# AlexIoannides/bodywork-mlops-demo

Hardware: NVIDIA H100
Metric: train rows/sec (N x 128 least-squares fit) (higher is better)
Workload: dtype bf16x2 (hi+lo) MMA operands, f32 accumulate, f64 fold+solve

## Files before the change

bodywork-mlops-demo_b200/csrc/b2_internal.cuh:

```cuda
#pragma once
#include <cuda.h>
#include <cuda_bf16.h>
#include <cuda_runtime.h>
#include <stdint.h>
#include <stdio.h>
#include <string.h>

#include <type_traits>

#include "../../include/b2gram.h"

namespace b2 {

constexpr int kMaxD = B2_MAX_D;
constexpr int kMaxS = kMaxD + 2;
constexpr int kKernelEventPairs = 64;
constexpr int kMaxRanks = 8;
constexpr size_t kXchgSlotDoubles = (size_t)kMaxS * kMaxS;
constexpr size_t kXchgDataDoubles = 2 * kMaxRanks * kXchgSlotDoubles;
constexpr size_t kXchgBytes = kXchgDataDoubles * sizeof(double) + 256;

constexpr int kTcRows = 64;
constexpr int kTcM = 128;
constexpr int kTcEMax = 16;
// ... 108 lines not shown
constexpr int kLcYbar = kLcC + kMaxD * kMaxClasses;
constexpr int kLcSum = kLcYbar + kMaxClasses;
constexpr int kLcPart = 2 * kMaxAlphas;
constexpr int kLcDoubles = kLcSum + kLcPart;

constexpr int kMnHead = 32;
constexpr int kMnClasses = 0;
constexpr int kMnCoef = kMaxClasses;
constexpr int kMnStep = kMnCoef + kMaxClasses * (kMaxD + 1);
constexpr int kMnOpDoubles = kMnStep + kMaxClasses * (kMaxD + 1);

constexpr int kDaHead = 8;
constexpr int kDaPart = kDaHead + kMaxD * kMaxD;
constexpr int kDaClasses = 0;
constexpr int kDaWeights = kMaxClasses;
constexpr int kDaMeans = 2 * kMaxClasses;
constexpr int kDaSums = kDaMeans + kMaxClasses * kMaxD;
constexpr int kDaDoubles = kDaSums + kDaPart;

constexpr int kQdClasses = 0;
constexpr int kQdMeans = kMaxClasses;
constexpr int kQdConst = kQdMeans + kMaxClasses * kMaxD;
constexpr int kQdW = kQdConst + kMaxClasses;
constexpr int kQdSums = kQdW + kMaxClasses * kMaxD * kMaxD;
constexpr int kQdCounts = kQdSums + kMaxClasses * kMaxD * kMaxD;
constexpr int kQdDoubles = kQdCounts + kMaxClasses + 8;
constexpr int64_t kQdSpan = 1 << 24;
constexpr int kQdChunk = 8192;
constexpr int kQdMaxChunks = (int)(kQdSpan / kQdChunk);
constexpr size_t kQdScratchBytes = sizeof(int) * (size_t)kQdSpan;
constexpr int kQdItemsPerSm = 2;
constexpr int kQdHdCorrect = 0;
constexpr int kQdHdNItems = 4;
constexpr int kQdHdCounts = 5;
constexpr int kQdHdStart = 8;
constexpr int kQdHdFirstItem = kQdHdStart + kMaxClasses + 1;
constexpr int kQdHdCnt = 80;
constexpr int kQdHdItems = kQdHdCnt + kQdMaxChunks * (kMaxClasses + 3);
static_assert(kQdHdFirstItem + kMaxClasses + 1 <= kQdHdCnt, "qda header");
int qda_max_items(const b2_ctx* ctx);

constexpr int kMaxFolds = 254;
int launch_fold_ranges(b2_ctx* ctx, const uint8_t* fold_of_row, int64_t n, int n_folds, unsigned long long* range);
int launch_fold_sum(b2_ctx* ctx, const double* folds, int n_folds, int d, double* S);

inline int narrow_dp(int d) { return d <= 1 ? 1 : d <= 2 ? 2 : d <= 4 ? 4 : d <= 8 ? 8 : 16; }

void set_error(const char* fmt, ...);

#define B2_CUDA(call)                                                                      \
  do {                                                                                     \
    cudaError_t e_ = (call);                                                               \
    if (e_ != cudaSuccess) {                                                               \
      b2::set_error("%s failed: %s (%s:%d)", #call, cudaGetErrorString(e_), __FILE__, __LINE__); \
      return B2_E_CUDA;                                                                    \
    }                                                                                      \
  } while (0)

}

struct b2_ctx {
  int device = 0;
  int sm_count = 0;
  size_t hbm_bytes = 0;
  char name[128] = {0};
  cudaStream_t stream = nullptr;
  cudaStream_t copy_stream = nullptr;
  cudaEvent_t ev_t0 = nullptr, ev_t1 = nullptr;
  cudaEvent_t ev_k[b2::kKernelEventPairs][2];
  int k_pairs = 0;
  int64_t launches = 0;

  int kernel_mode = B2_KERNEL_AUTO;
  int drain_rows = 8192;
  int precision = B2_PRECISION_SPLIT;

  int d = 0;
  double* S = nullptr;

  double* tc_part = nullptr;
  double* tc_red = nullptr;
  float* shift = nullptr;
  bool solve_attr_set = false;
  double* solve_host = nullptr;
  struct TmCache {
    const void* X = nullptr; const float* y = nullptr; const uint8_t* mask = nullptr;
    int64_t n = 0, ldx = 0; int d = 0, x_dtype = -1;
    int y_map_2d = 0, m_map_2d = 0;
    alignas(64) unsigned char tmX[128], tmY[128], tmM[128];
  } tm_cache;
  double* simt_part = nullptr;
  int simt_ctas = 0;
  double* score_part = nullptr;
  int score_ctas = 0;
  double* coef_dev = nullptr;
  double* grad_part = nullptr;
  double* refine = nullptr;
  double* loo = nullptr;
  double* loo_part = nullptr;
  double* enet = nullptr;
  size_t enet_doubles = 0;
  double* folds = nullptr;
  size_t folds_doubles = 0;
  int n_folds = 0;
  int folds_d = 0;
  unsigned long long* fold_range = nullptr;
  double* glm = nullptr;
  double* glm_part = nullptr;
  double* cls = nullptr;
  double* loo_cls = nullptr;
  double* mn_op = nullptr;
  double* mn_sum = nullptr;
  size_t mn_sum_doubles = 0;
  double* mn_part = nullptr;
  size_t mn_part_doubles = 0;
  double* disc = nullptr;
  double* disc_part = nullptr;
  double* qda = nullptr;
  int* qda_hd = nullptr;
  void* qda_scratch = nullptr;
  double* qda_part = nullptr;
  double* coef_host = nullptr;
  cudaEvent_t ev_coef[2] = {nullptr, nullptr};
  int coef_slot = 0;
  long long* synth_count = nullptr;
  double* solve_out = nullptr;
  void* stage_x[2] = {nullptr, nullptr};
  float* stage_y[2] = {nullptr, nullptr};
  uint8_t* stage_m[2] = {nullptr, nullptr};
  size_t stage_bytes_x = 0;
  int64_t stage_rows = 0;
  cudaEvent_t ev_copied[2] = {nullptr, nullptr};
  cudaEvent_t ev_consumed[2] = {nullptr, nullptr};
  bool ev_consumed_valid[2] = {false, false};
  char* row_out[2] = {nullptr, nullptr};
  size_t row_out_bytes = 0;
  void* bounce[2] = {nullptr, nullptr};
  cudaEvent_t ev_bounce[2] = {nullptr, nullptr};
  bool s_zero_pending = false;
  void* comm = nullptr;
  int n_ranks = 1, rank = 0;
  double* xchg = nullptr;
  double* xchg_peer[8] = {nullptr};
  bool p2p_ready = false;
  bool p2p_local = false;
  unsigned int xchg_epoch = 0;
  unsigned long long xchg_timeout_ns = 10000000000ull;
  bool xchg_pending = false;
  unsigned int* xchg_status_host = nullptr;
  unsigned int* tc_sync = nullptr;
  int fused_fits = 0;
  int sm_limit = 0;
  bool sm_limit_auto = false;
};

namespace b2 {

inline double* score_totals(const b2_ctx* ctx) { return ctx->score_part + (size_t)ctx->score_ctas * kNStats; }

template <typename... P, typename... A>
int launch_smem(void (*kernel)(P...), int grid, int threads, uint32_t smem, cudaStream_t stream, A... args) {
  B2_CUDA(cudaFuncSetAttribute(kernel, cudaFuncAttributeMaxDynamicSharedMemorySize, smem));
  kernel<<<grid, threads, smem, stream>>>(args...);
  B2_CUDA(cudaGetLastError());
  return B2_OK;
}
// ... 123 lines not shown
```

bodywork-mlops-demo_b200/csrc/gram_tc.cu:

```cuda
#include <cuda_bf16.h>
#include <stdlib.h>

#include "b2_internal.cuh"
#include "b2_ptx.cuh"
#include "b2_shift.cuh"
#include "b2_xchg.cuh"

namespace b2 {
namespace {

constexpr int kConsumerWGs = 2;
constexpr int kXformWarps = 8;
constexpr int kThreads = 128 * (kConsumerWGs + 2);
constexpr int kFirstXformWarp = 4 * kConsumerWGs;
constexpr int kTmaWarp = kFirstXformWarp;
constexpr int kEWarp = kFirstXformWarp + 1;
static_assert(kFirstXformWarp + kXformWarps == kThreads / 32, "warp roles");
constexpr int kProducers = kXformWarps;
constexpr int kConsumerWarps = 4 * kConsumerWGs;
constexpr int kKGroups = kTcRows / 8;
constexpr uint32_t kRawStageBytes = kTcRows * kMaxD * 4;
constexpr uint32_t kOpSBO = 128;
constexpr uint32_t kOpLBO = (16 + 2 + 16) * kOpSBO;
constexpr uint32_t kOpEOff = 16 * kOpSBO;
// ... 265 lines not shown
  auto P = [&](int acc, int i, int j) { return __ldcg(red + tc_part_index(acc, i, j, ew)); };
  auto s1 = [&](int i) {
    double t = 0.0;
    for (int blk = 0; blk < pack; ++blk) {
      const int r = blk * d + i, e = kTcM + 3 * blk;
      t += d2 ? P(0, r, e) + P(1, r, e) : P(0, r, e);
    }
    return t;
  };
  auto sxy = [&](int i) {
    double t = 0.0;
    for (int blk = 0; blk < pack; ++blk) {
      const int r = blk * d + i, e = kTcM + 3 * blk;
      t += d2 ? P(0, r, e + 1) + P(0, r, e + 2) + P(1, r, e + 1) + P(1, r, e + 2) : P(0, r, e + 1) + P(0, r, e + 2);
    }
    return t;
  };
  auto G = [&](int i, int j) {
    double g = 0.0;
    for (int blk = 0; blk < pack; ++blk) {
      const int ia = blk * d + i, ib = blk * d + j;
      const double g1 = P(0, min(ia, ib), max(ia, ib));
      g += d2 ? g1 + P(1, ia, ib) + P(1, ib, ia) : g1;
    }
    return g;
  };
  return unshift_entry(a, b, d, c, G, s1, sxy, __ldcg(red + kTcAccElems + 2), __ldcg(red + kTcAccElems + 0),
                       __ldcg(red + kTcAccElems + 1));
}

template <typename T, int DFIX, bool SPLIT, bool RAWB = false, int EW = 8>
__global__ void __launch_bounds__(kThreads, 1)
gram_tc_kernel(const __grid_constant__ CUtensorMap tmX, const __grid_constant__ CUtensorMap tmY,
               const __grid_constant__ CUtensorMap tmM, int y_map_2d, int has_mask, int keep,
               int64_t n_rows, int d_arg, int pack, int d_orig, const float* __restrict__ shift,
               int chunk_tiles, double* __restrict__ part, uint32_t wait_ns, uint32_t dbg_arg) {
#ifdef B2_DEV_KNOBS
  const uint32_t dbg = dbg_arg;
#else
  constexpr uint32_t dbg = 0u;
  (void)dbg_arg;
#endif
  using G = TcGeo<RAWB>;
  constexpr int kRawStages = G::kRawStages, kOpStages = G::kOpStages;
  constexpr uint32_t kOffRaw = G::kOffRaw, kOffOp = G::kOffOp, kOffY = G::kOffY, kOffMask = G::kOffMask;
  const int d = DFIX ? DFIX : d_arg;
  extern __shared__ uint8_t smem_raw[];
  const uint32_t sbase = (smem_u32(smem_raw) + 1023u) & ~1023u;
  uint8_t* smem = smem_raw + (sbase - smem_u32(smem_raw));
  const int warp = threadIdx.x >> 5;
  const int lane = threadIdx.x & 31;

  const uint32_t bar_raw_full = sbase + G::kOffBar;
  const uint32_t bar_raw_empty = bar_raw_full + 8 * kRawStages;
  const uint32_t bar_op_full = bar_raw_empty + 8 * kRawStages;
  const uint32_t bar_op_empty = bar_op_full + 8 * kOpStages;
  float* shift_s = reinterpret_cast<float*>(smem + G::kOffShift);

  const int64_t total_tiles = (n_rows + kTcRows - 1) / kTcRows;
  const int64_t tile_begin = (int64_t)blockIdx.x * total_tiles / gridDim.x;
  const int64_t tile_end = (int64_t)(blockIdx.x + 1) * total_tiles / gridDim.x;
  const int my_tiles = (int)(tile_end - tile_begin);

  if (threadIdx.x == 0) {
    for (int s = 0; s < kRawStages; ++s) {
      mbar_init(bar_raw_full + 8 * s, 1);
      mbar_init(bar_raw_empty + 8 * s, kProducers + (RAWB ? kConsumerWarps : 0));
    }
    for (int s = 0; s < kOpStages; ++s) {
      mbar_init(bar_op_full + 8 * s, kProducers);
      mbar_init(bar_op_empty + 8 * s, kConsumerWarps);
    }
    asm volatile("fence.mbarrier_init.release.cluster;" ::: "memory");
  }
  if (warp == kTmaWarp && lane == 0) {
    tma_prefetch_desc(&tmX);
    tma_prefetch_desc(&tmY);
    if (has_mask) tma_prefetch_desc(&tmM);
  }
  for (uint32_t o = threadIdx.x * 16; o < kOpStages * kOpStageBytes; o += kThreads * 16)
    *reinterpret_cast<uint4*>(smem + kOffOp + o) = make_uint4(0, 0, 0, 0);
  for (int j = threadIdx.x; j <= kMaxD; j += kThreads)
    shift_s[j] = j == kMaxD ? shift[kMaxD] : (j < pack * d_orig ? shift[j % d_orig] : 0.f);
  fence_proxy_async_smem();
  __syncthreads();

  if (warp < kConsumerWarps) {
    asm volatile("setmaxnreg.inc.sync.aligned.u32 %0;" ::"n"(G::kConsumerRegs));
    auto consume = [&](auto wg_c) {
      constexpr int WG = decltype(wg_c)::value;
      constexpr int kF1 = kTcM - 64 * WG;
      constexpr int kF2 = RAWB ? kF1 : kTcM;
      constexpr int kC1 = 64 * WG;
      constexpr int kR1 = (kF1 + EW) / 2, kR2 = (kF2 + EW) / 2;
      float acc1[kR1], acc2[kR2];
      using H = TcSums<DFIX, SPLIT, RAWB, EW, WG>;
      double* my_part = part + (size_t)blockIdx.x * kTcAccElems;
      double sums[H::kRegs > 0 ? H::kRegs : 1];
      const bool on_chip_off = (dbg & 256u) != 0u;
      auto slab_addr = [&](int s, int ln) {
        return sbase + G::kOffSlab + (uint32_t)(((4 * H::kSlabBase + (warp & 3) * H::kSlab + s) * 32 + ln) * 8);
      };
      auto store = [&](auto n_regs, int dst_acc, int col0, bool add, auto val) {
        const int ln = (int)lane_id(), row0 = 64 * WG + 16 * (warp & 3) + (ln >> 2);
#pragma unroll
        for (int r = 0; r < decltype(n_regs)::value; ++r) {
          const int col = col0 + 8 * (r >> 2) + 2 * (ln & 3) + (r & 1), h = (r >> 1) & 1, i = row0 + 8 * h;
          const bool lower = dst_acc == 0 && col < kTcM && i > col;
          const double v = val(r, col, h);
          const bool on_chip = dst_acc == 0 && r >= H::kFirstSlab;
          if (on_chip && r >= H::kFirstReg) {
            double& s = sums[r - H::kFirstReg];
            s = add ? __dadd_rn(s, v) : v;
          } else if (on_chip) {
            const uint32_t a = slab_addr(r - H::kFirstSlab, ln);
            st_shared_f64_if(a, add ? __dadd_rn(ld_shared_f64(a), v) : v, !on_chip_off);
          }
          put_f64(my_part + tc_part_index(dst_acc, i, col, EW), v, add, !lower && (!on_chip || on_chip_off));
        }
      };
      auto flush = [&]() {
        const int ln = (int)lane_id(), row0 = 64 * WG + 16 * (warp & 3) + (ln >> 2);
#pragma unroll
        for (int r = H::kFirstSlab; r < H::kR1; ++r) {
          const int col = kC1 + 8 * (r >> 2) + 2 * (ln & 3) + (r & 1), i = row0 + 8 * ((r >> 1) & 1);
          const double s = r >= H::kFirstReg ? sums[r - H::kFirstReg] : ld_shared_f64(slab_addr(r - H::kFirstSlab, ln));
          put_f64(my_part + tc_part_index(0, i, col, EW), s, false, !(col < kTcM && i > col) && !on_chip_off);
        }
      };
      auto drain = [&](const auto& acc, int dst_acc, int col0, bool add) {
        constexpr int kR = sizeof(acc) / sizeof(float);
        if constexpr (RAWB) {
          constexpr int kF = 2 * kR - EW;
          const double s1[2] = {(double)__shfl_sync(0xffffffffu, acc[kF / 2], lane & ~3),
                                (double)__shfl_sync(0xffffffffu, acc[kF / 2 + 2], lane & ~3)};
          store(std::integral_constant<int, kR>{}, dst_acc, col0, add, [&](int r, int col, int h) {
            return col < kTcM ? (double)acc[r] - (double)shift_s[col] * s1[h] : (double)acc[r];
          });
        } else {
          store(std::integral_constant<int, kR>{}, dst_acc, col0, add, [&](int r, int, int) { return (double)acc[r]; });
        }
      };
      auto release = [&](int tile) {
        mbar_arrive(bar_op_empty + 8 * (tile % kOpStages));
        if constexpr (RAWB) mbar_arrive(bar_raw_empty + 8 * (tile % kRawStages));
      };
      constexpr uint32_t a_off = (uint32_t)WG * 8 * kOpSBO;
      int os = 0, held = -1, in_chunk = 0;
      uint32_t oph = 0;
      bool first_chunk = true;
      for (int it = 0; it < my_tiles; ++it) {
        mbar_wait(bar_op_full + 8 * os, oph, wait_ns);
        const uint32_t op_addr = sbase + kOffOp + os * kOpStageBytes;
        wgmma_fence();
#pragma unroll
        for (int k2 = 0; k2 < kTcRows / 16; ++k2) {
          const uint32_t k_addr = op_addr + k2 * 2 * kOpLBO;
          const uint64_t hi_desc = make_smem_desc(k_addr + a_off), lo_desc = make_smem_desc(k_addr + kOpLoOff + a_off);
          const uint32_t sc1 = (in_chunk > 0 || k2 > 0) ? 1u : 0u, sc2 = (it > 0 || k2 > 0) ? 1u : 0u;
          if constexpr (RAWB) {
            const uint64_t x_desc = make_raw_desc(sbase + kOffRaw + (uint32_t)(it % kRawStages) * kRawStageBytes +
                                                  (uint32_t)WG * kRawBoxBytes + k2 * 16 * 128);
            const uint64_t e_desc = make_smem_desc(k_addr + kOpEOff);
            if (!(dbg & 2u)) {
              wgmma<kF1, 1>(acc1, hi_desc, x_desc, sc1);
              wgmma<EW, 0>(acc1 + kF1 / 2, hi_desc, e_desc, sc1);
            }
            if (SPLIT && !(dbg & 3u)) {
              wgmma<kF2, 1>(acc2, lo_desc, x_desc, sc2);
              wgmma<EW, 0>(acc2 + kF2 / 2, lo_desc, e_desc, sc2);
            }
          } else {
            if (!(dbg & 2u)) wgmma<kF1 + EW, 0>(acc1, hi_desc, make_smem_desc(k_addr + a_off), sc1);
            if (SPLIT && !(dbg & 3u)) wgmma<kF2 + EW, 0>(acc2, lo_desc, make_smem_desc(k_addr), sc2);
          }
        }
        wgmma_commit();
        const bool last = (in_chunk == chunk_tiles - 1) || (it == my_tiles - 1);
        if (last) {
          wgmma_wait<0>();
          fence_regs(acc1);
          if constexpr (SPLIT) fence_regs(acc2);
        } else {
          wgmma_wait<1>();
        }
        if (lane == 0) {
          if (held >= 0) release(held);
          if (last) release(it);
        }
        held = last ? -1 : it;
        if (last) {
          drain(acc1, 0, kC1, !first_chunk);
          first_chunk = false;
          in_chunk = 0;
        } else {
          ++in_chunk;
        }
        if (++os == kOpStages) { os = 0; oph ^= 1; }
      }
      wgmma_wait<0>();
      if constexpr (SPLIT) {
        fence_regs(acc2);
        drain(acc2, RAWB ? 0 : 1, RAWB ? kC1 : 0, RAWB);
      }
      flush();
    };
    if (__shfl_sync(0xffffffffu, warp, 0) >= 4) consume(std::integral_constant<int, 1>{});
    else consume(std::integral_constant<int, 0>{});
  } else {
    asm volatile("setmaxnreg.dec.sync.aligned.u32 %0;" ::"n"(G::kProducerRegs));
    const uint32_t tx = (uint32_t)(kTcRows * d * sizeof(T)) + kTcRows * pack * 4 + (has_mask ? kTcRows * pack : 0);
    auto issue = [&](int j) {
      const int s = j % kRawStages;
      mbar_wait(bar_raw_empty + 8 * s, ((uint32_t)(j / kRawStages) & 1u) ^ 1u, wait_ns);
      const uint32_t full = bar_raw_full + 8 * s;
      mbar_expect_tx(full, tx);
      const int64_t row0 = (tile_begin + j) * kTcRows;
      tma_load_2d(sbase + kOffRaw + s * kRawStageBytes, &tmX, 0, (int)row0, full);
      if constexpr (RAWB) tma_load_2d(sbase + kOffRaw + s * kRawStageBytes + kRawBoxBytes, &tmX, 64, (int)row0, full);
      const int sub0 = (int)row0 * pack;
      if (y_map_2d) tma_load_2d(sbase + kOffY + s * kYStageBytes, &tmY, 0, sub0 >> 2, full);
      else tma_load_1d(sbase + kOffY + s * kYStageBytes, &tmY, sub0, full);
      if (has_mask == 2) tma_load_2d(sbase + kOffMask + s * kMStageBytes, &tmM, 0, sub0 >> 4, full);
      else if (has_mask) tma_load_1d(sbase + kOffMask + s * kMStageBytes, &tmM, sub0, full);
    };
    const bool issuer = warp == kTmaWarp && lane == 0;
    if (issuer)
      for (int j = 0; j < G::kAhead && j < my_tiles; ++j) issue(j);

    const int t = warp - kFirstXformWarp;
    const int nb = (d + 63) >> 6;
    const int i = 64 * (t % nb) + 2 * lane;
    const uint32_t swp = ((uint32_t)lane >> 2) & 1u;
    const uint32_t st_off = (uint32_t)((i >> 3) * kOpSBO + (i & 7) * 16);
    auto esum = [&]() { return sbase + G::kOffESum + 8 * lane_id(); };
    if (warp == kEWarp) { st_shared_f64(esum(), 0.0); st_shared_f64(esum() + 256, 0.0); st_shared_f64(esum() + 512, 0.0); }
    int rs = 0, os = 0;
    uint32_t rph = 0, oph = 0;
    for (int it = 0; it < my_tiles; ++it) {
      if (issuer && it + G::kAhead < my_tiles) issue(it + G::kAhead);
      __syncwarp();
      mbar_wait(bar_raw_full + 8 * rs, rph, wait_ns);
      mbar_wait(bar_op_empty + 8 * os, oph ^ 1, wait_ns);
      const int64_t row0 = (tile_begin + it) * kTcRows;
      const int64_t left = n_rows - row0;
      const int rows_valid = left < kTcRows ? (int)left : kTcRows;
      const bool full_tile = (!has_mask) && (rows_valid == kTcRows);
      const uint32_t raw_addr = sbase + kOffRaw + rs * kRawStageBytes;
      const uint32_t m_addr = sbase + kOffMask + rs * kMStageBytes;
      const uint32_t op_addr = sbase + kOffOp + os * kOpStageBytes;
      if (warp == kEWarp && !(dbg & 192u)) {
        const uint32_t y_addr = sbase + kOffY + rs * kYStageBytes;
        const uint32_t e_addr = op_addr + kOpEOff;
        const float c_y = shift_s[kMaxD];
        float a = 0.f, b = 0.f, c = 0.f;
        for (int half = 0; half < kTcRows / 32; ++half) {
          const int rr = lane + 32 * half;
          const uint32_t dst = e_addr + (rr >> 3) * kOpLBO + (rr & 7) * 2;
          for (int bl = 0; bl < pack; ++bl) {
            const int sub = rr * pack + bl;
            bool use = rr < rows_valid;
            if (use && has_mask) use = (ld_shared_u8(m_addr + sub) == (uint32_t)keep);
            const float yv = use ? ld_shared_f32(y_addr + sub * 4) - c_y : 0.f;
            uint32_t yh, yl;
            split2(yv, 0.f, yh, yl);
            st_shared_u16(dst + (3 * bl) * 16, use ? 0x3F80u : 0u);
            st_shared_u16(dst + (3 * bl + 1) * 16, yh);
            st_shared_u16(dst + (3 * bl + 2) * 16, yl);
            if (RAWB && has_mask && !use) {
              const uint32_t row = raw_addr + (uint32_t)rr * 128;
              const uint32_t z[4] = {0u, 0u, 0u, 0u};
#pragma unroll
              for (int q = 0; q < 8; ++q) { st_shared_v4(row + 16 * q, z); st_shared_v4(row + kRawBoxBytes + 16 * q, z); }
            }
            a += yv;
            b = fmaf(yv, yv, b);
            c += use ? 1.f : 0.f;
          }
        }
        const uint32_t es = esum();
        st_shared_f64(es, ld_shared_f64(es) + (double)a);
        st_shared_f64(es + 256, ld_shared_f64(es + 256) + (double)b);
        st_shared_f64(es + 512, ld_shared_f64(es + 512) + (double)c);
      }
      if (i < d && !(dbg & 128u)) {
        float c_i[2];
        ld_vals_vec<float, 2>(sbase + G::kOffShift + 4 * (uint32_t)i, c_i);
        for (int g = t / nb; g < kKGroups; g += kXformWarps / nb) {
          const int r0 = g * 8;
          float v0[8], v1[8];
          const uint32_t src = raw_addr + (uint32_t)r0 * ((uint32_t)d * sizeof(T)) + (uint32_t)i * sizeof(T);
// ... 213 lines not shown
    if (pack > kMaxPack) pack = kMaxPack;
    if (n_in < (int64_t)2 * kTcRows * pack) pack = 1;
  }
  const int group = pack == 1 ? 1 : (pack == 3 ? 48 : (pack == 5 ? 80 : 16));
  if (pack_out != nullptr) *pack_out = pack;
  return n_in - n_in % group;
}

int launch_gram_tc(b2_ctx* ctx, const void* X, int x_dtype, const float* y, int64_t n_in, int d_in, int64_t ldx_in,
                   const uint8_t* mask, int keep, bool assign, unsigned int scatter_epoch) {
  PFN_encodeTiled encode = get_encode();
  if (encode == nullptr) {
    set_error("cuTensorMapEncodeTiled is not available from the driver");
    return B2_E_CUDA;
  }
  const int es = x_dtype == B2_F32 ? 4 : 2;
  int pack = 1;
  const int64_t n_main = gram_tc_main_rows(n_in, d_in, ldx_in, &pack);
  const int64_t n = n_main / pack;
  const int d = pack > 1 ? 128 : d_in;
  const int d_tensor = d_in * pack;
  const int64_t ldx = ldx_in * pack;
  const int64_t n_y = n_main;
  const bool rawb = x_dtype == B2_BF16 && d_in == 128 && pack == 1;
  CUtensorMap tmX, tmY, tmM;
  b2_ctx::TmCache& tc = ctx->tm_cache;
  const bool cached = tc.X == X && tc.y == y && tc.mask == mask && tc.n == n_in && tc.ldx == ldx_in && tc.d == d_in &&
                      tc.x_dtype == x_dtype;
  if (cached) {
    memcpy(&tmX, tc.tmX, sizeof(tmX)); memcpy(&tmY, tc.tmY, sizeof(tmY)); memcpy(&tmM, tc.tmM, sizeof(tmM));
  } else {
    int y_map_2d = 0, m_map_2d = 0;
    if (int r = encode_maps(encode, X, x_dtype, es, y, n, d_tensor, d, ldx, n_y, pack, mask, rawb, &tmX, &tmY, &tmM, &y_map_2d,
                            &m_map_2d))
      return r;
    tc.X = X; tc.y = y; tc.mask = mask; tc.n = n_in; tc.ldx = ldx_in; tc.d = d_in; tc.x_dtype = x_dtype;
    tc.y_map_2d = y_map_2d; tc.m_map_2d = m_map_2d;
    memcpy(tc.tmX, &tmX, sizeof(tmX)); memcpy(tc.tmY, &tmY, sizeof(tmY)); memcpy(tc.tmM, &tmM, sizeof(tmM));
  }

  const int64_t total_tiles = (n + kTcRows - 1) / kTcRows;
  const int sms = (ctx->sm_limit > 0 && ctx->sm_limit < ctx->sm_count) ? ctx->sm_limit : ctx->sm_count;
  const int grid = (int)(total_tiles < sms ? total_tiles : sms);
  int chunk_tiles = ctx->drain_rows / kTcRows / (rawb ? 4 : 1);
  if (chunk_tiles < 1) chunk_tiles = 1;

#ifdef B2_DEV_KNOBS
  static const uint32_t wait_ns = []() {
    const char* e = getenv("B2_WAIT_HINT_NS");
    return e ? (uint32_t)atoi(e) : 20000u;
  }();
#else
  constexpr uint32_t wait_ns = 20000u;
#endif
#ifdef B2_DEV_KNOBS
  static const uint32_t dbg = []() {
    const char* e = getenv("B2_TC_DEBUG");
    return e ? (uint32_t)atoi(e) : 0u;
  }();
#else
  constexpr uint32_t dbg = 0u;
#endif
  const bool split = ctx->precision == B2_PRECISION_SPLIT;
  const int ew = tc_e_width(pack);
  const bool d2 = split && !rawb;
  decltype(&gram_tc_kernel<float, 0, false>) kernel = nullptr;
  uint32_t smem = TcGeo<false>::kSmemBytes;
  with_rows(x_dtype, X, [&](auto* Xr) {
    using T = row_t<decltype(Xr)>;
    return with_int<0, 1>(split, [&](auto SP) {
      constexpr bool kSplit = decltype(SP)::value;
      if (d != 128) kernel = gram_tc_kernel<T, 0, kSplit>;
      else if (ew == 16) kernel = gram_tc_kernel<T, 128, kSplit, false, 16>;
      else kernel = gram_tc_kernel<T, 128, kSplit>;
      if constexpr (std::is_same_v<T, __nv_bfloat16>) {
        if (rawb) {
          kernel = gram_tc_kernel<T, 128, kSplit, true>;
          smem = TcGeo<true>::kSmemBytes;
        }
      }
      return B2_OK;
    });
  });
  B2_CUDA(cudaFuncSetAttribute(kernel, cudaFuncAttributeMaxDynamicSharedMemorySize, smem));
  const int pair = ctx->k_pairs % kKernelEventPairs;
  B2_CUDA(cudaEventRecord(ctx->ev_k[pair][0], ctx->stream));
  kernel<<<grid, kThreads, smem, ctx->stream>>>(tmX, tmY, tmM, tc.y_map_2d, mask != nullptr ? 1 + tc.m_map_2d : 0, keep,
                                                n, d, pack, d_in, ctx->shift, chunk_tiles, ctx->tc_part, wait_ns, dbg);
  B2_CUDA(cudaGetLastError());
  B2_CUDA(cudaEventRecord(ctx->ev_k[pair][1], ctx->stream));
  ctx->k_pairs += 1;

  TcFinal fin;
  memset(&fin, 0, sizeof(fin));
  fin.assign = assign ? 1 : 0;
  fin.n_ranks = 1;
  if (scatter_epoch != 0) {
    fin.n_ranks = ctx->n_ranks; fin.rank = ctx->rank; fin.epoch = scatter_epoch;
    for (int r = 0; r < kMaxRanks; ++r) fin.peers.p[r] = ctx->xchg_peer[r];
  }
  {
    cudaLaunchConfig_t cfg;
    memset(&cfg, 0, sizeof(cfg));
    cfg.gridDim = dim3(kFinalizeCtas < sms ? kFinalizeCtas : sms);
    cfg.blockDim = dim3(kFinalizeThreads); cfg.dynamicSmemBytes = 0; cfg.stream = ctx->stream;
    cudaLaunchAttribute attr[1];
    attr[0].id = cudaLaunchAttributeCooperative;
    attr[0].val.cooperative = 1;
    cfg.attrs = attr; cfg.numAttrs = 1;
    const double* part_arg = ctx->tc_part;
    const float* shift_arg = ctx->shift;
    B2_CUDA(cudaLaunchKernelEx(&cfg, tc_finalize_kernel, part_arg, grid, ctx->tc_red, shift_arg, d_in, pack, ew,
                               d2 ? 1 : 0, ctx->S, ctx->tc_sync, fin));
  }
  ctx->launches += 2;
  return B2_OK;
}

}
```

bodywork-mlops-demo_b200/csrc/solve.cu:

```cuda
#include "b2_internal.cuh"
#include "b2_xchg.cuh"

namespace b2 {
namespace {

constexpr int kOutIntercept = kMaxD;
constexpr int kOutInfo = kMaxD + 1;
constexpr int kOutRank = kMaxD + 2;
constexpr int kOutSingular = kMaxD + 3;
constexpr int kOutRows = kOutSingular + kMaxD;

struct LdcgStat {
  const double* S;
  __device__ __forceinline__ double operator()(int i) const { return __ldcg(S + i); }
};

template <class Stat>
__device__ void build_normal_equations_of(const Stat& S, int d, double alpha, int fit_intercept,
                                       double* A, double* r, double* mean, double* ybar_out) {
  const int dp = d + 2, pitch = d + 1;
  const double n = S(d * dp + d);
  const double inv_n = n > 0.0 ? 1.0 / n : 0.0;
  double sxy = 0.0;
  if ((int)threadIdx.x < d) {
    const double sx = S(threadIdx.x * dp + d);
    sxy = S(threadIdx.x * dp + d + 1);
    mean[threadIdx.x] = fit_intercept ? sx * inv_n : 0.0;
  }
  const double ybar = fit_intercept ? S(d * dp + d + 1) * inv_n : 0.0;
  __syncthreads();
  if ((int)threadIdx.x < d) r[threadIdx.x] = sxy - n * mean[threadIdx.x] * ybar;
  const int lane = threadIdx.x & 31, warp = threadIdx.x >> 5, nwarps = blockDim.x >> 5;
  for (int i0 = warp; i0 < d; i0 += 2 * nwarps) {
    const int i1 = i0 + nwarps;
    double v[8];
#pragma unroll
    for (int u = 0; u < 4; ++u) {
      const int j = lane + 32 * u;
      v[u] = j < d ? S(i0 * dp + j) : 0.0;
      v[4 + u] = (j < d && i1 < d) ? S(i1 * dp + j) : 0.0;
    }
    const double m0 = mean[i0], m1 = i1 < d ? mean[i1] : 0.0;
#pragma unroll
    for (int u = 0; u < 4; ++u) {
      const int j = lane + 32 * u;
      if (j < d) {
        const double mj = mean[j];
        A[i0 * pitch + j] = v[u] - n * m0 * mj + (i0 == j ? alpha : 0.0);
        if (i1 < d) A[i1 * pitch + j] = v[4 + u] - n * m1 * mj + (i1 == j ? alpha : 0.0);
      }
    }
  }
  if (threadIdx.x == 0) *ybar_out = ybar;
  __syncthreads();
}

__device__ __forceinline__ void build_normal_equations(const double* S, int d, double alpha, int fit_intercept,
                                                       double* A, double* r, double* mean, double* ybar_out) {
  build_normal_equations_of(LdcgStat{S}, d, alpha, fit_intercept, A, r, mean, ybar_out);
}

__device__ __forceinline__ double rcp_pos(double x) {
  double y;
  asm("rcp.approx.ftz.f64 %0, %1;" : "=d"(y) : "d"(x));
  const double er = fma(-x, y, 1.0);
  const double t = fma(er, er, er);
  return fma(y, t, y);
}

struct SolveXchg {
  double* own;
  int n_ranks;
  unsigned int epoch;
  unsigned long long timeout_ns;
};

constexpr int kNB = 16;
constexpr int kCholThreads = 512;
constexpr int kUPitch = kNB + 1;

__device__ void refine_update(const double* S, int d, int fit_intercept, bool singular, const double* dbeta, double* misc,
                              double* __restrict__ rf, double* __restrict__ out);

template <bool REFINE>
__global__ void __launch_bounds__(kCholThreads, 1)
solve_cholesky_kernel(double* S, int d, double alpha, int fit_intercept, double* __restrict__ out, const SolveXchg xc,
                      double* __restrict__ rf) {
  extern __shared__ double sm[];
  const int pitch = d + 1;
  double* A = sm;
  double* r = A + d * pitch;
  double* mean = A + (d + 1) * pitch;
  double* invd = mean + d;
  double* misc = invd + d;
  double* U = misc + 8;
  const int tid = threadIdx.x, lane = tid & 31;
  const int warp = __shfl_sync(0xffffffffu, tid >> 5, 0);
  long long tm[5] = {0, 0, 0, 0, 0};
  long long tc0 = clock64();
  if (xc.own != nullptr) {
    __shared__ int ok;
    if (tid == 0) ok = xchg_wait(xc.own, xc.n_ranks, xc.epoch, xc.timeout_ns) ? 1 : 0;
    __syncthreads();
    if (!ok) {
      if (tid == 0) {
        xchg_flags(xc.own)[kXchgStatusWord] = xc.epoch;
        out[kOutInfo] = -1.0;
      }
      return;
    }
    const int dp = d + 2;
    for (int base = 0; base < dp * dp; base += 4 * blockDim.x) {
      double sv[4];
#pragma unroll
      for (int u = 0; u < 4; ++u) {
        const int idx = base + u * blockDim.x + tid;
        sv[u] = idx < dp * dp ? xchg_sum(xc.own, xc.n_ranks, xc.epoch, idx) : 0.0;
      }
#pragma unroll
      for (int u = 0; u < 4; ++u) {
        const int idx = base + u * blockDim.x + tid;
        if (idx < dp * dp) S[idx] = sv[u];
      }
    }
    __threadfence();
    __syncthreads();
  }
  build_normal_equations(S, d, alpha, fit_intercept, A, r, mean, &misc[0]);
  if constexpr (REFINE) {
    if (tid < d) r[tid] = rf[kRfGrad + tid] - alpha * rf[kRfBeta + tid];
    __syncthreads();
  }
  tm[0] = clock64() - tc0;
  if (warp == 0) {
    double mx = 0.0;
    for (int i = lane; i < d; i += 32) mx = fmax(mx, A[i * pitch + i]);
#pragma unroll
    for (int o = 16; o > 0; o >>= 1) mx = fmax(mx, __shfl_xor_sync(0xffffffffu, mx, o));
    if (lane == 0) { misc[1] = mx; misc[2] = 0.0; }
  }
  __syncthreads();
  const double tiny = misc[1] * 1e-12;
  const int rows = d + 1;

  for (int kb = 0; kb < d; kb += kNB) {
    const int nb = (d - kb) < kNB ? (d - kb) : kNB;
    tc0 = clock64();
    if (warp == 0) {
      const int lrow = lane & (kNB - 1), h = lane >> 4;
      const bool act = lrow < nb;
      const int row = kb + (act ? lrow : 0);
      double a[kNB / 2];
#pragma unroll
      for (int cc = 0; cc < kNB / 2; ++cc) {
        const int c = 2 * cc + h;
        a[cc] = (act && c < nb) ? A[row * pitch + kb + c] : 0.0;
      }
      double my_rc = 1.0;
      int first_bad = 0;
#pragma unroll
      for (int k = 0; k < kNB; ++k) {
        if (k < nb) {
          const int hk = k & 1, kk = k >> 1;
          const double colk = a[kk];
          const double piv = __shfl_sync(0xffffffffu, colk, k | (hk << 4));
          const bool bad = !(piv > tiny);
          const double rc = bad ? 1.0 : rcp_pos(piv);
          const double u = __shfl_sync(0xffffffffu, colk, lrow | (hk << 4));
          my_rc = (lrow == k) ? rc : my_rc;
          first_bad = (bad && first_bad == 0) ? (kb + k + 1) : first_bad;
#pragma unroll
          for (int cc = 0; cc < kNB / 2; ++cc) {
            if (2 * cc + 1 > k) {
              const int c = 2 * cc + h;
              const double uc = __shfl_sync(0xffffffffu, colk, c | (hk << 4));
              if (c > k) a[cc] = fma(-(u * uc), rc, a[cc]);
            }
          }
          if (h == hk && act && lrow > k) {
            A[row * pitch + kb + k] = u * rc;
            U[row * kUPitch + k] = u;
          }
        }
      }
      if (act && h == 0) invd[kb + lrow] = my_rc;
      if (lane == 0 && first_bad != 0 && misc[2] == 0.0) misc[2] = (double)first_bad;
    }
    __syncthreads();
    tm[1] += clock64() - tc0; tc0 = clock64();
    if (misc[2] != 0.0) break;
    {
      const int prow = tid >> 2, q = tid & 3;
      const int below = rows - kb - nb;
      const bool live = prow < below;
      const int i = kb + nb + (live ? prow : 0);
      double sv[4];
#pragma unroll
      for (int j = 0; j < 4; ++j) {
        const int c = 4 * j + q;
        sv[j] = (live && c < nb) ? A[i * pitch + kb + c] : 0.0;
      }
      const int qbase = lane & ~3;
      double rinv[kNB];
#pragma unroll
      for (int m = 0; m < kNB; ++m) rinv[m] = m < nb ? invd[kb + m] : 0.0;
      double out_m[4], out_u[4];
#pragma unroll
      for (int j = 0; j < 4; ++j) { out_m[j] = 0.0; out_u[j] = 0.0; }
#pragma unroll
      for (int m = 0; m < kNB; ++m) {
        if (m < nb) {
          const double um = __shfl_sync(0xffffffffu, sv[m >> 2], qbase | (m & 3));
          const double xm = um * rinv[m];
          if (q == (m & 3)) { out_m[m >> 2] = xm; out_u[m >> 2] = um; }
#pragma unroll
          for (int j = 0; j < 4; ++j) {
            if (4 * j + 3 > m) {
              const int c = 4 * j + q;
              if (c > m && c < nb) sv[j] = fma(-xm, U[(kb + c) * kUPitch + m], sv[j]);
            }
          }
        }
      }
      if (live) {
#pragma unroll
        for (int j = 0; j < 4; ++j) {
          const int m = 4 * j + q;
          if (m < nb) { A[i * pitch + kb + m] = out_m[j]; U[i * kUPitch + m] = out_u[j]; }
        }
      }
    }
    __syncthreads();
    tm[2] += clock64() - tc0; tc0 = clock64();
    {
      const int base = kb + nb;
      const int nti = (rows - base + 7) >> 3, ntj = (d - base + 7) >> 3;
      const int tri = ntj * (ntj + 1) / 2;
      const int total = tri + (nti > ntj ? ntj : 0);
      const int g = lane >> 2, t4 = lane & 3;
      constexpr int kWarps = kCholThreads / 32, kInFlight = 4;
      for (int t0 = warp; t0 < total; t0 += kWarps * kInFlight) {
        int ia[kInFlight], jb[kInFlight];
        double c0[kInFlight], c1[kInFlight], av[kInFlight][kNB / 4], bv[kInFlight][kNB / 4];
#pragma unroll
        for (int f = 0; f < kInFlight; ++f) {
          const int t = t0 + f * kWarps;
          int ti = 0, tj = 0;
          if (t < tri) {
            ti = (int)((sqrtf(8.0f * (float)t + 1.0f) - 1.0f) * 0.5f);
            while (ti * (ti + 1) / 2 > t) --ti;
            while ((ti + 1) * (ti + 2) / 2 <= t) ++ti;
            tj = t - ti * (ti + 1) / 2;
          } else if (t < total) {
            ti = ntj; tj = t - tri;
          }
          const bool live = t < total;
          ia[f] = live ? base + 8 * ti + g : rows;
          jb[f] = live ? base + 8 * tj + g : d;
#pragma unroll
          for (int sgm = 0; sgm < kNB / 4; ++sgm) {
            const int m = 4 * sgm + t4;
            av[f][sgm] = (ia[f] < rows && m < nb) ? -A[ia[f] * pitch + kb + m] : 0.0;
            bv[f][sgm] = (jb[f] < d && m < nb) ? U[jb[f] * kUPitch + m] : 0.0;
          }
          c0[f] = 0.0; c1[f] = 0.0;
        }
#pragma unroll
        for (int sgm = 0; sgm < kNB / 4; ++sgm) {
#pragma unroll
          for (int f = 0; f < kInFlight; ++f)
            asm volatile("mma.sync.aligned.m8n8k4.row.col.f64.f64.f64.f64 {%0, %1}, {%2}, {%3}, {%0, %1};"
                         : "+d"(c0[f]), "+d"(c1[f]) : "d"(av[f][sgm]), "d"(bv[f][sgm]));
        }
#pragma unroll
        for (int f = 0; f < kInFlight; ++f) {
          const int jc = jb[f] - g + 2 * t4;
          if (ia[f] < rows) {
            if (jc < d) A[ia[f] * pitch + jc] += c0[f];
            if (jc + 1 < d) A[ia[f] * pitch + jc + 1] += c1[f];
          }
        }
      }
    }
    __syncthreads();
    tm[3] += clock64() - tc0;
  }
  tc0 = clock64();
  const bool singular = misc[2] != 0.0;
  if (!singular) {
    for (int kb = ((d - 1) / kNB) * kNB; kb >= 0; kb -= kNB) {
      const int nb = (d - kb) < kNB ? (d - kb) : kNB;
      if (warp == 0) {
        const int col = lane & (kNB - 1);
        const bool act = lane < nb;
        double lt[kNB];
#pragma unroll
        for (int k = 0; k < kNB; ++k) lt[k] = (act && k < nb && k > col) ? A[(kb + k) * pitch + kb + col] : 0.0;
        double z = act ? r[kb + col] : 0.0;
#pragma unroll
        for (int k = kNB - 1; k >= 0; --k) {
          if (k < nb) {
            const double bk = __shfl_sync(0xffffffffu, z, k);
            z = (lane < k) ? fma(-lt[k], bk, z) : z;
          }
        }
        __syncwarp();
        if (act) r[kb + lane] = z;
      }
      __syncthreads();
      for (int i = tid; i < kb; i += blockDim.x) {
        double acc0 = 0.0, acc1 = 0.0;
#pragma unroll
        for (int m = 0; m < kNB; m += 2) {
          if (m < nb) acc0 = fma(A[(kb + m) * pitch + i], r[kb + m], acc0);
          if (m + 1 < nb) acc1 = fma(A[(kb + m + 1) * pitch + i], r[kb + m + 1], acc1);
        }
        r[i] -= acc0 + acc1;
      }
      __syncthreads();
    }
  }
  tm[4] = clock64() - tc0;
  if constexpr (REFINE) {
    refine_update(S, d, fit_intercept, singular, r, misc, rf, out);
    return;
  }
  if (tid == 0)
    for (int k = 0; k < 5; ++k) out[kOutSingular + k] = (double)tm[k];
  for (int i = tid; i < d; i += blockDim.x) out[i] = singular ? 0.0 : r[i];
  if (warp == 0) {
    double part = 0.0;
    for (int i = lane; i < d; i += 32) part += mean[i] * r[i];
#pragma unroll
    for (int o = 16; o > 0; o >>= 1) part += __shfl_xor_sync(0xffffffffu, part, o);
    if (lane == 0) {
      out[kOutIntercept] = singular ? 0.0 : misc[0] - part;
      out[kOutInfo] = misc[2];
    }
  }
}

__device__ void refine_update(const double* S, int d, int fit_intercept, bool singular, const double* dbeta, double* misc,
                              double* __restrict__ rf, double* __restrict__ out) {
  const int tid = threadIdx.x, lane = tid & 31, warp = tid >> 5;
  const int dp = d + 2;
// ... 1190 lines not shown
  }
}

constexpr int kClsThreads = 512;
size_t solve_classes_smem_bytes(int d, int n_targets) {
  return sizeof(double) * ((size_t)(d + n_targets) * (d + 1) + 3 * kMaxD + kMaxClasses + 16);
}

__global__ void __launch_bounds__(kClsThreads, 1)
solve_classes_kernel(double* S, int d, double alpha, int fit_intercept, int n_classes, double* __restrict__ cls) {
  extern __shared__ double sm[];
  const int T = n_classes == 2 ? 1 : n_classes, pitch = d + 1, rows = d + T;
  double* A = sm;
  double* mean = A + rows * pitch;
  double* tot = mean + kMaxD;
  double* col = tot + kMaxD;
  double* misc = col + kMaxD + kMaxClasses;
  const double* sums = cls + kClsSums;
  const int tid = threadIdx.x, lane = tid & 31, warp = tid >> 5, nwarps = blockDim.x >> 5;
  build_normal_equations(S, d, alpha, fit_intercept, A, A + d * pitch, mean, &misc[0]);
  const double n = __ldcg(S + d * (d + 2) + d);
  if (tid < d) {
    double s = 0.0;
    for (int k = 0; k < n_classes; ++k) s += sums[k * (d + 1) + tid];
    tot[tid] = s;
  }
  __syncthreads();
  for (int t = tid; t < T * d; t += blockDim.x) {
    const int tt = t / d, j = t - tt * d, k = T == 1 ? 1 : tt;
    const double sk = sums[k * (d + 1) + j], nk = sums[k * (d + 1) + d];
    A[(d + tt) * pitch + j] = fit_intercept ? 2.0 * (sk - (nk / n) * tot[j]) : 2.0 * sk - tot[j];
  }
  if (warp == 0) {
    double mx = 0.0;
    for (int i = lane; i < d; i += 32) mx = fmax(mx, A[i * pitch + i]);
#pragma unroll
    for (int o = 16; o > 0; o >>= 1) mx = fmax(mx, __shfl_xor_sync(0xffffffffu, mx, o));
    if (lane == 0) misc[1] = mx;
  }
  __syncthreads();
  const double tiny = misc[1] * 1e-12;
  int info = 0;
  for (int k = 0; k < d; ++k) {
    const double piv = A[k * pitch + k];
    if (!(piv > tiny)) { info = k + 1; break; }
    const double rc = 1.0 / piv;
    for (int i = k + 1 + tid; i < rows; i += blockDim.x) col[i] = A[i * pitch + k];
    __syncthreads();
    for (int i = k + 1 + warp; i < rows; i += nwarps) {
      const double f = col[i] * rc;
      const int jend = i < d ? i : d - 1;
      for (int j = k + 1 + lane; j <= jend; j += 32) A[i * pitch + j] = fma(-f, col[j], A[i * pitch + j]);
      if (lane == 0) A[i * pitch + k] = f;
    }
    __syncthreads();
  }
  for (int t = warp; t < T; t += nwarps) {
    double* z = A + (d + t) * pitch;
    if (info == 0) {
      for (int i = d - 1; i > 0; --i) {
        const double wi = z[i];
        for (int m = lane; m < i; m += 32) z[m] = fma(-A[i * pitch + m], wi, z[m]);
        __syncwarp();
      }
    }
    double part = 0.0;
    for (int j = lane; j < d; j += 32) {
      const double w = info == 0 ? z[j] : 0.0;
      cls[kClsCoef + t * kMaxD + j] = w;
      part = fma(mean[j], w, part);
    }
#pragma unroll
    for (int o = 16; o > 0; o >>= 1) part += __shfl_xor_sync(0xffffffffu, part, o);
    if (lane == 0) {
      const int k = T == 1 ? 1 : t;
      const double ybar = fit_intercept ? 2.0 * sums[k * (d + 1) + d] / n - 1.0 : 0.0;
      cls[kClsIntercept + t] = info == 0 ? ybar - part : 0.0;
    }
  }
  if (tid == 0) cls[kClsInfo] = (double)info;
}

size_t solve_smem_bytes(int d) {
  const size_t chol = (size_t)(d + 1) * (d + 1) + 3 * d + 16 + (size_t)(d + 1) * kUPitch;
  const size_t eig = (size_t)(d + 1) * (d + 1) + 3 * d + 16 + 4 * kMaxD + kMaxD + 2 * (kMaxD + 8) + kMaxD;
  return sizeof(double) * (chol > eig ? chol : eig);
}

int ensure_solve_attrs(b2_ctx* ctx) {
  if (!ctx->solve_attr_set) {
    const int bytes = (int)solve_smem_bytes(kMaxD);
    B2_CUDA(cudaFuncSetAttribute(solve_cholesky_kernel<false>, cudaFuncAttributeMaxDynamicSharedMemorySize, bytes));
    B2_CUDA(cudaFuncSetAttribute(solve_cholesky_kernel<true>, cudaFuncAttributeMaxDynamicSharedMemorySize, bytes));
    B2_CUDA(cudaFuncSetAttribute(solve_spectral_kernel, cudaFuncAttributeMaxDynamicSharedMemorySize, bytes));
    B2_CUDA(cudaFuncSetAttribute(solve_eigvals_kernel, cudaFuncAttributeMaxDynamicSharedMemorySize, bytes));
    B2_CUDA(cudaFuncSetAttribute(solve_eigh_kernel, cudaFuncAttributeMaxDynamicSharedMemorySize,
                                 (int)eigh_smem_bytes(kMaxD)));
    B2_CUDA(cudaFuncSetAttribute(solve_enet_kernel, cudaFuncAttributeMaxDynamicSharedMemorySize,
                                 (int)enet_smem_bytes(kMaxD)));
    B2_CUDA(cudaFuncSetAttribute(bayes_ridge_kernel, cudaFuncAttributeMaxDynamicSharedMemorySize,
                                 (int)bayes_smem_bytes(kMaxD)));
    B2_CUDA(cudaFuncSetAttribute(ard_kernel, cudaFuncAttributeMaxDynamicSharedMemorySize, (int)ard_smem_bytes(kMaxD)));
    ctx->solve_attr_set = true;
  }
  return B2_OK;
}

}

int launch_solve_cholesky(b2_ctx* ctx, double alpha, int fit_intercept, unsigned int gather_epoch) {
  if (int r = ensure_solve_attrs(ctx)) return r;
  SolveXchg xc;
  xc.own = gather_epoch != 0 ? ctx->xchg : nullptr;
  xc.n_ranks = ctx->n_ranks;
  xc.epoch = gather_epoch;
  xc.timeout_ns = ctx->xchg_timeout_ns;
  solve_cholesky_kernel<false><<<1, kCholThreads, solve_smem_bytes(ctx->d), ctx->stream>>>(ctx->S, ctx->d, alpha,
                                                                                           fit_intercept, ctx->solve_host,
                                                                                           xc, nullptr);
  B2_CUDA(cudaGetLastError());
  ctx->launches += 1;
  return B2_OK;
}

int launch_solve_classes(b2_ctx* ctx, double alpha, int fit_intercept, int n_classes) {
  const int T = n_classes == 2 ? 1 : n_classes;
  if (int r = launch_smem(solve_classes_kernel, 1, kClsThreads, (uint32_t)solve_classes_smem_bytes(ctx->d, T),
                          ctx->stream, ctx->S, ctx->d, alpha, fit_intercept, n_classes, ctx->cls))
    return r;
  ctx->launches += 1;
  return B2_OK;
}

int launch_solve_refine(b2_ctx* ctx, double alpha, int fit_intercept) {
  if (int r = ensure_solve_attrs(ctx)) return r;
  SolveXchg xc;
  xc.own = nullptr;
  xc.n_ranks = 1;
  xc.epoch = 0;
  xc.timeout_ns = 0;
  solve_cholesky_kernel<true><<<1, kCholThreads, solve_smem_bytes(ctx->d), ctx->stream>>>(ctx->S, ctx->d, alpha,
                                                                                          fit_intercept, ctx->solve_host,
                                                                                          xc, ctx->refine);
  B2_CUDA(cudaGetLastError());
  ctx->launches += 1;
  return B2_OK;
}

int launch_solve_spectral(b2_ctx* ctx, double cond, int fit_intercept) {
  if (int r = ensure_solve_attrs(ctx)) return r;
  solve_spectral_kernel<<<1, 512, solve_smem_bytes(ctx->d), ctx->stream>>>(ctx->S, ctx->d, cond, fit_intercept, ctx->solve_out);
  B2_CUDA(cudaGetLastError());
  ctx->launches += 1;
  return B2_OK;
}

int launch_solve_eigh(b2_ctx* ctx, int fit_intercept) {
  if (int r = ensure_solve_attrs(ctx)) return r;
  solve_eigh_kernel<<<1, kEighThreads, eigh_smem_bytes(ctx->d), ctx->stream>>>(ctx->S, ctx->d, fit_intercept, ctx->loo);
  B2_CUDA(cudaGetLastError());
  ctx->launches += 1;
  return B2_OK;
}

int launch_solve_enet(b2_ctx* ctx, const EnetArgs& args) {
  if (int r = ensure_solve_attrs(ctx)) return r;
  const int ctas = args.folds != nullptr ? args.n_folds * args.n_l1 : 1;
// ... 33 lines not shown
```

Before: 5.492 billion.

## Cache gram kernel smem attribute, pad Cholesky panel, add negated panel copy

Skips the per-call cudaFuncSetAttribute on the gram kernel by recording in the context which kernel instantiations already have it set. In the blocked Cholesky trailing update, a negated copy of the panel is stored in a padded shared-memory buffer (pitch 20 instead of 17), so the f64 MMA operand loads read a contiguous, conflict-reduced array instead of strided A with a negation. It also adds globaltimer per-CTA printf instrumentation, compiled only under B2_DEV_KNOBS. The cost is extra shared memory for the solve kernel and extra stores when the panel is written.

Measured after the change: 5.510 billion (median of 6 runs). About the same (+0.3%).

```diff
diff --git a/bodywork-mlops-demo_b200/csrc/b2_internal.cuh b/bodywork-mlops-demo_b200/csrc/b2_internal.cuh
--- a/bodywork-mlops-demo_b200/csrc/b2_internal.cuh
+++ b/bodywork-mlops-demo_b200/csrc/b2_internal.cuh
@@ -214,6 +214,7 @@
   double* tc_red = nullptr;
   float* shift = nullptr;
   bool solve_attr_set = false;
+  const void* tc_attr_set[16] = {};
   double* solve_host = nullptr;
   struct TmCache {
     const void* X = nullptr; const float* y = nullptr; const uint8_t* mask = nullptr;
diff --git a/bodywork-mlops-demo_b200/csrc/gram_tc.cu b/bodywork-mlops-demo_b200/csrc/gram_tc.cu
--- a/bodywork-mlops-demo_b200/csrc/gram_tc.cu
+++ b/bodywork-mlops-demo_b200/csrc/gram_tc.cu
@@ -371,8 +371,16 @@
     *reinterpret_cast<uint4*>(smem + kOffOp + o) = make_uint4(0, 0, 0, 0);
   for (int j = threadIdx.x; j <= kMaxD; j += kThreads)
     shift_s[j] = j == kMaxD ? shift[kMaxD] : (j < pack * d_orig ? shift[j % d_orig] : 0.f);
+#ifdef B2_DEV_KNOBS
+  __shared__ unsigned int dbg_done;
+  if (threadIdx.x == 0) dbg_done = 0u;
+#endif
   fence_proxy_async_smem();
   __syncthreads();
+#ifdef B2_DEV_KNOBS
+  unsigned long long dbg_t0 = 0ull;
+  if (dbg & 512u) asm volatile("mov.u64 %0, %%globaltimer;" : "=l"(dbg_t0));
+#endif
 
   if (warp < kConsumerWarps) {
     asm volatile("setmaxnreg.inc.sync.aligned.u32 %0;" ::"n"(G::kConsumerRegs));
@@ -496,6 +504,16 @@
     };
     if (__shfl_sync(0xffffffffu, warp, 0) >= 4) consume(std::integral_constant<int, 1>{});
     else consume(std::integral_constant<int, 0>{});
+#ifdef B2_DEV_KNOBS
+    if (dbg & 512u) {
+      __syncwarp();
+      if (lane == 0 && atomicAdd(&dbg_done, 1u) == (unsigned int)kConsumerWarps - 1u) {
+        unsigned long long t1;
+        asm volatile("mov.u64 %0, %%globaltimer;" : "=l"(t1));
+        printf("[gram_cta] %d %llu %llu\n", (int)blockIdx.x, dbg_t0, t1);
+      }
+    }
+#endif
   } else {
     asm volatile("setmaxnreg.dec.sync.aligned.u32 %0;" ::"n"(G::kProducerRegs));
     const uint32_t tx = (uint32_t)(kTcRows * d * sizeof(T)) + kTcRows * pack * 4 + (has_mask ? kTcRows * pack : 0);
@@ -875,7 +893,14 @@
       return B2_OK;
     });
   });
-  B2_CUDA(cudaFuncSetAttribute(kernel, cudaFuncAttributeMaxDynamicSharedMemorySize, smem));
+  bool attr_set = false;
+  for (const void*& k : ctx->tc_attr_set) {
+    if (k == nullptr) k = reinterpret_cast<const void*>(kernel);
+    else if (k != reinterpret_cast<const void*>(kernel)) continue;
+    else attr_set = true;
+    break;
+  }
+  if (!attr_set) B2_CUDA(cudaFuncSetAttribute(kernel, cudaFuncAttributeMaxDynamicSharedMemorySize, smem));
   const int pair = ctx->k_pairs % kKernelEventPairs;
   B2_CUDA(cudaEventRecord(ctx->ev_k[pair][0], ctx->stream));
   kernel<<<grid, kThreads, smem, ctx->stream>>>(tmX, tmY, tmM, tc.y_map_2d, mask != nullptr ? 1 + tc.m_map_2d : 0, keep,
diff --git a/bodywork-mlops-demo_b200/csrc/solve.cu b/bodywork-mlops-demo_b200/csrc/solve.cu
--- a/bodywork-mlops-demo_b200/csrc/solve.cu
+++ b/bodywork-mlops-demo_b200/csrc/solve.cu
@@ -77,7 +77,7 @@
 
 constexpr int kNB = 16;
 constexpr int kCholThreads = 512;
-constexpr int kUPitch = kNB + 1;
+constexpr int kUPitch = kNB + 4;
 
 __device__ void refine_update(const double* S, int d, int fit_intercept, bool singular, const double* dbeta, double* misc,
                               double* __restrict__ rf, double* __restrict__ out);
@@ -94,6 +94,7 @@
   double* invd = mean + d;
   double* misc = invd + d;
   double* U = misc + 8;
+  double* Mn = U + (d + 1) * kUPitch;
   const int tid = threadIdx.x, lane = tid & 31;
   const int warp = __shfl_sync(0xffffffffu, tid >> 5, 0);
   long long tm[5] = {0, 0, 0, 0, 0};
@@ -226,7 +227,11 @@
 #pragma unroll
         for (int j = 0; j < 4; ++j) {
           const int m = 4 * j + q;
-          if (m < nb) { A[i * pitch + kb + m] = out_m[j]; U[i * kUPitch + m] = out_u[j]; }
+          if (m < nb) {
+            A[i * pitch + kb + m] = out_m[j];
+            U[i * kUPitch + m] = out_u[j];
+            Mn[i * kUPitch + m] = -out_m[j];
+          }
         }
       }
     }
@@ -260,7 +265,7 @@
 #pragma unroll
           for (int sgm = 0; sgm < kNB / 4; ++sgm) {
             const int m = 4 * sgm + t4;
-            av[f][sgm] = (ia[f] < rows && m < nb) ? -A[ia[f] * pitch + kb + m] : 0.0;
+            av[f][sgm] = (ia[f] < rows && m < nb) ? Mn[ia[f] * kUPitch + m] : 0.0;
             bv[f][sgm] = (jb[f] < d && m < nb) ? U[jb[f] * kUPitch + m] : 0.0;
           }
           c0[f] = 0.0; c1[f] = 0.0;
@@ -1617,7 +1622,7 @@
 }
 
 size_t solve_smem_bytes(int d) {
-  const size_t chol = (size_t)(d + 1) * (d + 1) + 3 * d + 16 + (size_t)(d + 1) * kUPitch;
+  const size_t chol = (size_t)(d + 1) * (d + 1) + 3 * d + 16 + 2 * (size_t)(d + 1) * kUPitch;
   const size_t eig = (size_t)(d + 1) * (d + 1) + 3 * d + 16 + 4 * kMaxD + kMaxD + 2 * (kMaxD + 8) + kMaxD;
   return sizeof(double) * (chol > eig ? chol : eig);
 }
```
